# PaiDii/TGTC-Style

Hardware: AMD Instinct MI355X
Metric: rays/sec (128c+64f samples) on fern 400x400 (higher is better)
Workload: dtype f16 MFMA product + two block-scaled fp6 (e2m3) correction products, f32 accumulate (fine pass; coarse pass: fp16x3); 1 GPU; fern-shaped 400x400 frame, plain NeRF render (style off), 128 coarse + 64 fine samples/ray, one whole frame per rank per step, seeded random-init weights; precision=fp16x3+fp16mx

## Files before the change

### tgtc-style_amd/csrc/mlp_nerf_fp16s.hip

```cpp
#define TGTC_ASM_DMA 1
#include "mlp_nerf_mx.h"

#include "mlp_layouts.h"

namespace tgtc {

#ifndef TGTC_FP16S_INC
#define TGTC_FP16S_INC "fp16s_asm_nerf.inc"
#endif
#include TGTC_FP16S_INC

using CfgFp16s = MlpCfg<4, kFp16sTiles, false, 4>;
#ifndef TGTC_FRONT_ABL
#define TGTC_FRONT_ABL 0
#endif

template <int IN_MODE>
__global__ void __launch_bounds__(256, 1) nerf_fp16s_kernel(NerfArgs a, long long n_pass) {
    using C = CfgFp16s;
    constexpr int NCT = C::NCT;
    using Ring = WeightStream<C, SingleStreamMap<NerfLayout::kFragsSigma>, true, true>;
    constexpr int kChunk = kFp16sChunkBytes, kSlots = C::RING_BYTES / kChunk, kLook = kSlots - 1, kPiece = kChunk / C::NWAVES;
    constexpr int kPad = ((NerfLayout::kFragsSigma * C::FRAG_BYTES + kChunk - 1) / kChunk + kSlots - 1) / kSlots * kSlots;
    static_assert(NerfLayout::kFragsSigma == kFp16sFrags && kPad == kFp16sPadChunks && C::RING_BYTES == 131072 && C::FRAG_BYTES == 1024 &&
                      kPiece % 4096 == 0 && kChunk == kChunkBytes,
                  "the generated stream was laid out for this ring");

    __shared__ __attribute__((aligned(16))) char smem[C::RING_BYTES + kNerfBiasBytes];
    const int wave = __builtin_amdgcn_readfirstlane(threadIdx.x >> 6);
    Ring ring;
    {
        const int lane = threadIdx.x & 63;
        const char* const streams[1] = {a.stream};
        ring.init(streams, smem, wave, lane);
#pragma unroll
        for (int j = 0; j < kNerfBiasBytes / (C::NWAVES * 1024); ++j)
            lds_dma16(a.bias + (j * C::NWAVES + wave) * 1024 + lane * 16, smem + C::RING_BYTES + (j * C::NWAVES + wave) * 1024);
        ring.lds_wave = smem + wave * kPiece;
        ring.voff = wave * kPiece + lane * 16;
        static_for<kLook * (kPiece / 1024)>([&](auto i_) {
            constexpr int i = decltype(i_)::value, ch = i / (kPiece / 1024), j = i % (kPiece / 1024);
            lds_dma16_s<(j % 4) * 1024>(ring.src[0] + ch * kChunk + (j / 4) * 4096, ring.voff, ring.lds_wave + ch * kChunk + (j / 4) * 4096);
        });
    }

    for (long long p = blockIdx.x; p < n_pass; p += gridDim.x) {
        const long long s_wave = p * C::SAMPLES_PER_WG + wave * C::SAMPLES_PER_WAVE;
        half8 keep[NCT][2];
        unsigned bad = 0;
        {
            const int lane = fresh_lane_id();
            const int g = lane >> 4, n = lane & 15;
            double pos[NCT][3], dir[NCT][3];
            long long sidx[NCT];
            half8 pe_h[2][NCT], pe_l[2][NCT], de_h[1][NCT], de_l[1][NCT];
#if TGTC_FRONT_ABL & 1
#pragma unroll
            for (int c = 0; c < NCT; ++c) pe_h[0][c] = pe_h[1][c] = half8{(_Float16)(float)(g + n)};
#else
            nerf_load_samples<NCT, IN_MODE>(a, s_wave, n, pos, dir, sidx);
            nerf_encode<NCT, false, false>(a, pos, dir, sidx, g, pe_h, pe_l, de_h, de_l);
#pragma unroll
            for (int c = 0; c < NCT; ++c)
                if (!(__builtin_isfinite(pos[c][0]) && __builtin_isfinite(pos[c][1]) && __builtin_isfinite(pos[c][2]))) bad |= 1u << c;
#endif
#pragma unroll
            for (int c = 0; c < NCT; ++c) keep[c][0] = pe_h[0][c], keep[c][1] = pe_h[1][c];
        }
        const int fl = fresh_lane_id();
        ring.voff = wave * kPiece + fl * 16;
        ring.lane_lo = opaque((lds_cptr)smem + fl * 16);
        ring.lane_hi = opaque((lds_cptr)smem + 65536 + fl * 16);
        const lds_cptr bias_lane = opaque((lds_cptr)smem + C::RING_BYTES + 16 * (fl >> 4));
        float sigma[NCT];
        fp16s_asm_nerf_sigma_pass(ring, bias_lane, keep, sigma);
        const int lane = fresh_lane_id();
        if (lane < 16) {
#pragma unroll
            for (int c = 0; c < NCT; ++c) {
                const long long s = s_wave + c * 16 + lane;
                if (s < a.M) a.sigma[s] = (bad >> c & 1) ? __builtin_nanf("") : sigma[c];
            }
        }
    }
    wait_vmcnt<0>();
}

int nerf_fp16s_launch(const NerfArgs& a, hipStream_t st) {
    using C = CfgFp16s;
    if (a.M <= 0) return TGTC_OK;
    if (a.M >= 0x7fffffffLL) return fail(TGTC_ERR_UNSUPPORTED, "nerf: too many samples in one launch (%lld)", a.M);
    int cus = 0;
    if (const int rc = cu_count(cus)) return rc;
    const long long n_pass = (a.M + C::SAMPLES_PER_WG - 1) / C::SAMPLES_PER_WG;
    nerf_fp16s_kernel<IN_RAYS><<<(unsigned)(n_pass < cus ? n_pass : cus), C::NWAVES * 64, 0, st>>>(a, n_pass);
    TGTC_LAUNCH_CHECK();
    return TGTC_OK;
}

}
```

Measured before the change: 3.103 million rays/s.

## Overlap next pass's sample load and encoding inside the sigma MLP stream

```diff
diff --git a/tgtc-style_amd/csrc/mlp_nerf_fp16s.hip b/tgtc-style_amd/csrc/mlp_nerf_fp16s.hip
--- a/tgtc-style_amd/csrc/mlp_nerf_fp16s.hip
+++ b/tgtc-style_amd/csrc/mlp_nerf_fp16s.hip
@@ -1,5 +1,7 @@
 #define TGTC_ASM_DMA 1
 #include "mlp_nerf_mx.h"
+
+#include <cstdlib>
 
 #include "mlp_layouts.h"
 
@@ -15,7 +17,34 @@
 #define TGTC_FRONT_ABL 0
 #endif
 
-template <int IN_MODE>
+__device__ __forceinline__ unsigned udiv_word(unsigned n) {
+    unsigned z = (unsigned)(__builtin_amdgcn_rcpf((float)n) * 4294966784.0f);
+    return z + __umulhi(z, (0u - n) * z);
+}
+
+template <int IN_MODE, int NCT>
+__device__ __forceinline__ void fp16s_front(const NerfArgs& a, long long s_wave, half8 (&keep)[NCT][2], unsigned& bad) {
+    const int lane = fresh_lane_id();
+    const int g = lane >> 4, n = lane & 15;
+    double pos[NCT][3], dir[NCT][3];
+    long long sidx[NCT];
+    half8 pe_h[2][NCT], pe_l[2][NCT], de_h[1][NCT], de_l[1][NCT];
+    bad = 0;
+#if TGTC_FRONT_ABL & 1
+#pragma unroll
+    for (int c = 0; c < NCT; ++c) pe_h[0][c] = pe_h[1][c] = half8{(_Float16)(float)(g + n)};
+#else
+    nerf_load_samples<NCT, IN_MODE>(a, s_wave, n, pos, dir, sidx);
+    nerf_encode<NCT, false, false>(a, pos, dir, sidx, g, pe_h, pe_l, de_h, de_l);
+#pragma unroll
+    for (int c = 0; c < NCT; ++c)
+        if (!(__builtin_isfinite(pos[c][0]) && __builtin_isfinite(pos[c][1]) && __builtin_isfinite(pos[c][2]))) bad |= 1u << c;
+#endif
+#pragma unroll
+    for (int c = 0; c < NCT; ++c) keep[c][0] = pe_h[0][c], keep[c][1] = pe_h[1][c];
+}
+
+template <int IN_MODE, bool FRONT>
 __global__ void __launch_bounds__(256, 1) nerf_fp16s_kernel(NerfArgs a, long long n_pass) {
     using C = CfgFp16s;
     constexpr int NCT = C::NCT;
@@ -25,6 +54,7 @@
     static_assert(NerfLayout::kFragsSigma == kFp16sFrags && kPad == kFp16sPadChunks && C::RING_BYTES == 131072 && C::FRAG_BYTES == 1024 &&
                       kPiece % 4096 == 0 && kChunk == kChunkBytes,
                   "the generated stream was laid out for this ring");
+    static_assert(!FRONT || IN_MODE == IN_RAYS, "the in-stream front end loads samples of rays");
 
     __shared__ __attribute__((aligned(16))) char smem[C::RING_BYTES + kNerfBiasBytes];
     const int wave = __builtin_amdgcn_readfirstlane(threadIdx.x >> 6);
@@ -44,36 +74,30 @@
         });
     }
 
+    unsigned bad = 0;
+    half8 keep[NCT][2];
+    if constexpr (FRONT) {
+        fp16s_front<IN_MODE>(a, (long long)blockIdx.x * C::SAMPLES_PER_WG + wave * C::SAMPLES_PER_WAVE, keep, bad);
+        fp16s_asm_first_keep(keep);
+    }
+    const unsigned mm1 = (unsigned)(a.M - 1), zz = __builtin_amdgcn_readfirstlane(udiv_word((unsigned)a.N));
+
     for (long long p = blockIdx.x; p < n_pass; p += gridDim.x) {
         const long long s_wave = p * C::SAMPLES_PER_WG + wave * C::SAMPLES_PER_WAVE;
-        half8 keep[NCT][2];
-        unsigned bad = 0;
-        {
-            const int lane = fresh_lane_id();
-            const int g = lane >> 4, n = lane & 15;
-            double pos[NCT][3], dir[NCT][3];
-            long long sidx[NCT];
-            half8 pe_h[2][NCT], pe_l[2][NCT], de_h[1][NCT], de_l[1][NCT];
-#if TGTC_FRONT_ABL & 1
-#pragma unroll
-            for (int c = 0; c < NCT; ++c) pe_h[0][c] = pe_h[1][c] = half8{(_Float16)(float)(g + n)};
-#else
-            nerf_load_samples<NCT, IN_MODE>(a, s_wave, n, pos, dir, sidx);
-            nerf_encode<NCT, false, false>(a, pos, dir, sidx, g, pe_h, pe_l, de_h, de_l);
-#pragma unroll
-            for (int c = 0; c < NCT; ++c)
-                if (!(__builtin_isfinite(pos[c][0]) && __builtin_isfinite(pos[c][1]) && __builtin_isfinite(pos[c][2]))) bad |= 1u << c;
-#endif
-#pragma unroll
-            for (int c = 0; c < NCT; ++c) keep[c][0] = pe_h[0][c], keep[c][1] = pe_h[1][c];
-        }
+        if constexpr (!FRONT) fp16s_front<IN_MODE>(a, s_wave, keep, bad);
         const int fl = fresh_lane_id();
         ring.voff = wave * kPiece + fl * 16;
         ring.lane_lo = opaque((lds_cptr)smem + fl * 16);
         ring.lane_hi = opaque((lds_cptr)smem + 65536 + fl * 16);
         const lds_cptr bias_lane = opaque((lds_cptr)smem + C::RING_BYTES + 16 * (fl >> 4));
         float sigma[NCT];
-        fp16s_asm_nerf_sigma_pass(ring, bias_lane, keep, sigma);
+        unsigned nbad = 0;
+        if constexpr (FRONT) {
+            const unsigned snext = (unsigned)(s_wave + (long long)gridDim.x * C::SAMPLES_PER_WG);
+            fp16s_asm_nerf_sigma_pass_front(ring, bias_lane, sigma, nbad, a.ts, a.rays_o, a.rays_d, mm1, (unsigned)a.N, zz, snext);
+        } else {
+            fp16s_asm_nerf_sigma_pass(ring, bias_lane, keep, sigma);
+        }
         const int lane = fresh_lane_id();
         if (lane < 16) {
 #pragma unroll
@@ -82,6 +106,7 @@
                 if (s < a.M) a.sigma[s] = (bad >> c & 1) ? __builtin_nanf("") : sigma[c];
             }
         }
+        if constexpr (FRONT) bad = nbad;
     }
     wait_vmcnt<0>();
 }
@@ -93,7 +118,10 @@
     int cus = 0;
     if (const int rc = cu_count(cus)) return rc;
     const long long n_pass = (a.M + C::SAMPLES_PER_WG - 1) / C::SAMPLES_PER_WG;
-    nerf_fp16s_kernel<IN_RAYS><<<(unsigned)(n_pass < cus ? n_pass : cus), C::NWAVES * 64, 0, st>>>(a, n_pass);
+    const unsigned grid = (unsigned)(n_pass < cus ? n_pass : cus);
+    const char* e = std::getenv("TGTC_SCREEN_SERIAL_FRONT");
+    if (e && e[0] == '1') nerf_fp16s_kernel<IN_RAYS, false><<<grid, C::NWAVES * 64, 0, st>>>(a, n_pass);
+    else nerf_fp16s_kernel<IN_RAYS, true><<<grid, C::NWAVES * 64, 0, st>>>(a, n_pass);
     TGTC_LAUNCH_CHECK();
     return TGTC_OK;
 }
```

Measured after the change: 3.164 million rays/s (median of 6 runs). 1.9% higher.
